# OpenResearchInstitute/ka9q-sdr

Hardware: AMD Instinct MI355X
Metric: input Msamples/s + channels @ real-time, 16384-pt overlap-save (higher is better)
Workload: dtype f32

## Files before the change

ka9q_sdr_amd/csrc/kq_bank.cpp:

```cpp
#include <cstdarg>

#include "kq_bank.hpp"

using namespace kq::bank;

namespace {
thread_local std::string g_err;

int ilog2(unsigned v) {
  int l = 0;
  while ((1u << l) < v) l++;
  return l;
}
}

void kq_internal_set_error(const char *fmt, ...) {
  char buf[512];
  va_list ap;
  va_start(ap, fmt);
  vsnprintf(buf, sizeof buf, fmt, ap);
  va_end(ap);
  g_err = buf;
}

// ... 235 lines not shown
      if (b->alloc(&h, C * (size_t)(g.Mdec > 1 ? g.Mdec - 1 : 1), true)) return -1;
  }
  if (b->alloc(&b->chd.foffset, C, true)) return -1;
  if (b->alloc(&b->chd.pdev, C, true)) return -1;
  if (b->alloc(&b->chd.gain, C, true)) return -1;
  if (b->alloc(&b->chd.hang, C, true)) return -1;
  if (b->alloc(&b->chd.dc, C, true)) return -1;
  if (b->alloc(&b->chd.n0, C, true)) return -1;
  if (b->alloc(&b->chd.pl_ptr, C, true)) return -1;
  if (b->alloc(&b->chd.pl_last, C, true)) return -1;
  if (b->alloc(&b->chd.plfreq, C, true)) return -1;
  if (g.pl_n > 0) {
    if (b->alloc(&b->chd.plresp, (size_t)g.pl_n / 2 + 1, true)) return -1;
    if (b->alloc(&b->chd.plring, C * 16384, true)) return -1;
  }
  if (b->alloc(&b->pl.audio, C * B * 2 * (size_t)g.olen, true)) return -1;
  if (b->alloc(&b->pl.status, C * B, true)) return -1;
  for (int k = 0; k < 2; k++) {
    b->pl2[k].audio = b->pl.audio;
    b->pl2[k].status = b->pl.status;
    if (b->alloc(&b->pl2[k].filt, C * B * g.olen, true)) return -1;
    if (b->alloc(&b->pl2[k].n0raw, C * B, true)) return -1;
    if (b->alloc(&b->pl2[k].if_power, B * (1 + kq::kEnergySplitMax), true)) return -1;
    if (g.pl_n > 0 && b->alloc(&b->pl2[k].plout, C * B * g.pl_l, true)) return -1;
  }
  b->pl = b->pl2[0];
  if (b->alloc(&b->energy_state, 2, true)) return -1;
  if (kq::full16k_paired_supported(g) && b->alloc(&b->win_paired, (size_t)(g.M - 1) + (size_t)B * g.L, true)) return -1;
  for (int *&l : b->list_dev)
    if (b->alloc(&l, C, true)) return -1;
  for (kq_bank::CtlQueue &q : b->ctl)
    for (int k = 0; k < kq_bank::CtlQueue::kDepth; k++)
      if (b->alloc_pinned(&q.buf[k], kq_bank::CtlQueue::kBytes) || b->new_event(&q.applied[k], hipEventDisableTiming)) return -1;
  {
    kq_bank::DesignQueue &d = b->dq;
    size_t const per_job = (size_t)g.Ndec * sizeof(float2);
    d.max_jobs = (unsigned)std::max<size_t>(1, std::min<size_t>(kq_bank::DesignQueue::kMax, ((size_t)64 << 20) / per_job));
    if (b->alloc(&d.scratch, (size_t)d.max_jobs * g.Ndec, true)) return -1;
    if (b->alloc(&d.ng_next, 2 * C, true)) return -1;
    for (int k = 0; k < kq_bank::DesignQueue::kDepth; k++)
      if (b->alloc_pinned(&d.pin[k], kq_bank::DesignQueue::kMax * (sizeof(kq::DesignJob) + sizeof(kq::DesignTarget))) ||
          b->new_event(&d.read[k], hipEventDisableTiming))
        return -1;
    for (hipEvent_t &e : d.ng_moved)
      if (b->new_event(&e, hipEventDisableTiming)) return -1;
    if (g.Ndec <= 16384 && kq::design_prepare(g.olen, g.Mdec)) return -1;
  }
  if (b->alloc(&b->list_active_dev, C, true)) return -1;
  if (b->alloc(&b->list_active_ds_dev, C, true)) return -1;
  if (b->alloc(&b->chd.fflags, C, true)) return -1;
  if (b->alloc(&b->list_unswept_dev, C, true)) return -1;
  if (b->alloc(&b->list_swept_dev, C, true)) return -1;
  if (b->fwd_mode == KQ_FWD_PRUNED && b->alloc(&b->chan_tw, C * kq::pruned_table_elems(g), true)) return -1;
  if (b->fwd_mode != KQ_FWD_PRUNED && kq::full16k_supported(g) && b->alloc(&b->chd.row_ph, C * 32, true)) return -1;
  KQ_TRY(hipStreamSynchronize(b->stream));
  if (g.pl_n > 0) {
    int const PL_M = g.pl_n - g.pl_l + 1;
    std::vector<kq::cfloat> r(g.pl_n / 2 + 1, kq::cfloat(0, 0));
    for (int j = 0; j <= g.pl_n / 2; j++) {
      float const f = (float)j * g.dsamprate / g.Ndec;
      if (f > 0 && f < 300) r[j] = 1;
    }
    if (kq::window_rfilter(g.pl_l, PL_M, r, 2.0)) return -1;
    KQ_TRY(hipMemcpy(b->chd.plresp, r.data(), r.size() * sizeof(float2), hipMemcpyHostToDevice));
  }
  {
    std::vector<float> nanv(C, NAN);
    KQ_TRY(hipMemcpy(b->chd.plfreq, nanv.data(), C * sizeof(float), hipMemcpyHostToDevice));
  }
  return 0;
}
}

kq_bank *kq_bank_create(const kq_bank_config *cfg) {
  if (create_check(cfg)) return nullptr;
  kq::DeviceScope dev_scope_(cfg->device);
  {
    int cur = -1;
    if (hipGetDevice(&cur) != hipSuccess || cur != cfg->device) {
      kq_internal_set_error("hipSetDevice(%d) failed", cfg->device);
      return nullptr;
    }
  }
  kq_bank *b = new kq_bank();
  b->cfg = *cfg;
  b->chans.reserve(cfg->max_channels);
  if (create_geometry(b) || create_alloc(b)) {
    kq_bank_destroy(b);
    return nullptr;
  }
  return b;
}

int kq_bank_destroy(kq_bank *b) {
  kq::DeviceScope dev_scope_(b ? b->cfg.device : -1);
  if (!b) return 0;
  b->close();
  delete b;
  return 0;
}

void *kq_bank_stream(kq_bank *b) { return b ? (void *)b->stream : nullptr; }

int kq_bank_join(kq_bank *b) {
  BankScope dev_scope_(b);
  if (!b) return -1;
  if (b->calls == 0) return 0;
// ... 59 lines not shown
```

ka9q_sdr_amd/csrc/kq_device.hpp:

```cpp
#pragma once
#include "kq_energy.hpp"
#include <hip/hip_runtime.h>
#include <stdint.h>

#include <functional>

#include "../../include/ka9q_hip.h"

struct filter_in;

namespace kq {

enum { FLAG_FLAT = 1, FLAG_ISB = 2, FLAG_STEREO = 4, FLAG_SQUARE = 8 };

struct PllState {
  double c_phase, c_freq;
  double f_phase, f_freq;
  float integrator, delta_f, snr, foffset, cphase;
  int lock_count, pll_lock, fft_samples, fft_ptr;
};

struct FftDim {
  int n;
  int log2n;
  int nf;
  unsigned char f[12];
  const unsigned short *rev;
  const float2 *twc;
  int tw_n;
};
FftDim fft_dim(int n, bool *ok);
bool fft_size_ok(int n);
const float2 *half_twiddles(int log2T);
enum { TABLE_HALF_TWIDDLES, TABLE_DIM_REV, TABLE_DIM_TW, TABLE_FULL16K };
const void *upload_once(int table, int size, size_t bytes, const std::function<void(void *)> &fill);

constexpr int kPllChunk = 64;
struct PllChunk {
  PllState *state;
  float2 *rings;
  float2 *side;
};

struct Geom {
  int N, L, M, D;
  FftDim dN, dNdec, dPl;
  int Ndec, olen, Mdec;
  int log2N, log2Ndec;
  int samprate;
  int tw_log2;
  int max_blocks;
  float dsamprate;
  int pl_n, pl_l;
};

constexpr int kOldLevels = 4;

struct ChanDev {
  int *mode;
  int *flags;
  int *fflags;
  float *low, *high;
  float2 *resp;
  float2 *aresp;
  float *fm_gain;
  float *headroom;
  float *recovery;
  int *hangmax;
  float *noise_gain;
  unsigned long long *n0lane;
  unsigned *n0meta;
  int *n0slot;
  double *lo_phase, *lo_freq, *lo_rate;
  float2 *row_ph;
  double *hist_phase, *hist_freq, *hist_rate;
  int *hist_len;
  int *hist2_len;
  double *hist2_osc;
  double *sh_phase, *sh_freq;
  float2 *fm_state;
  float *lastaudio;
  int *sq_count;
  float *ahist;
  float *foffset, *pdev;
  float *gain;
  int *hang;
  float *dc;
  float *n0;
  float2 *plresp;
  float *plring;
  int *pl_ptr, *pl_last;
  float *plfreq;
};

struct Planes {
  float2 *filt;
  float *audio;
  kq_chan_status *status;
  float *n0raw;
  float *if_power;
  float *plout;
};

struct DeviceScope {
  int prev = -1;
  bool switched = false;
  explicit DeviceScope(int device) {
    if (device < 0) return;
    if (hipGetDevice(&prev) == hipSuccess && prev != device) switched = hipSetDevice(device) == hipSuccess;
  }
  ~DeviceScope() {
    if (switched) (void)hipSetDevice(prev);
  }
  DeviceScope(const DeviceScope &) = delete;
  DeviceScope &operator=(const DeviceScope &) = delete;
};

void ensure_dynamic_lds(const void *kernel, size_t bytes);

void launch_copy_to_host(hipStream_t s, const float *audio, float *haudio, int row, const kq_chan_status *status, void *hstatus,
                         size_t rows);
void launch_copy_pcm_to_host(hipStream_t s, const float *audio, short *hpcm, unsigned *hmask, int row,
                             const kq_chan_status *status, void *hstatus, size_t rows, const int *mode_compact = nullptr,
                             int max_blocks = 1);
void launch_ingest(hipStream_t s, const void *src, int format, float2 *dst, size_t nsamples, float scale);
constexpr int kEnergySplitMax = 16;
int block_energy_split(int L);
// ... 68 lines not shown
```

ka9q_sdr_amd/csrc/kq_full16k.hip:

```cpp
#include "kq_device.hpp"
#include "kq_ldsfft.hpp"
#include <cmath>
#include <type_traits>

#include "kq_lane.hpp"
#include "kq_regfft.hpp"

#ifdef KQ_TIMELINE
__device__ unsigned long long kq_timeline[64][8][12];
#define KQ_STAMP(i)                                                                        \
  do {                                                                                     \
    __builtin_amdgcn_sched_barrier(0);                                                     \
    if (blockIdx.y == (gridDim.y > 40 ? 40 : gridDim.y / 2) && (blockIdx.x & 15) == 0 && (blockIdx.x >> 4) < 64 &&      \
        (threadIdx.x & 63) == 0)                                                           \
      kq_timeline[blockIdx.x >> 4][threadIdx.x >> 6][i] = clock64();                       \
    __builtin_amdgcn_sched_barrier(0);                                                     \
  } while (0)
extern "C" int kq_debug_timeline(unsigned long long *dst) {
  return hipMemcpyFromSymbol(dst, HIP_SYMBOL(kq_timeline), sizeof(kq_timeline)) == hipSuccess ? 0 : -1;
}
#else
#define KQ_STAMP(i)
#endif

namespace kq {

namespace {

constexpr int kN = 16384, kT = 512;
constexpr int kRow1 = 528;
constexpr int kCol2 = 32;
constexpr int kRow2 = 513;
constexpr int kXchElems = 16 * kRow1;

using rfft::pk_cmul;
using rfft::pk_cmul2;
using rfft::pk_cmul4;
using rfft::pk_cmul_s;
using rfft::v2f;

__device__ __forceinline__ v2f ld2(const float2 *p) {
  float2 const f = *p;
  return (v2f){f.x, f.y};
}

using rsrc_t = __amdgpu_buffer_rsrc_t;
__device__ __forceinline__ rsrc_t make_rsrc(const void *base, unsigned bytes) {
  return __builtin_amdgcn_make_buffer_rsrc(const_cast<void *>(base), 0, (int)bytes, 0x00020000);
}
__device__ __forceinline__ v2f buf_ld2(rsrc_t r, unsigned lane_off, unsigned row_off) {
  return __builtin_bit_cast(v2f, __builtin_amdgcn_raw_buffer_load_b64(r, (int)lane_off, (int)row_off, 0));
}
__device__ __forceinline__ void buf_ld4(v2f &a, v2f &b, rsrc_t r, unsigned lane_off, unsigned row_off) {
  typedef float v4f __attribute__((ext_vector_type(4)));
  v4f const q = __builtin_bit_cast(v4f, __builtin_amdgcn_raw_buffer_load_b128(r, (int)lane_off, (int)row_off, 0));
  a = (v2f){q.x, q.y};
  b = (v2f){q.z, q.w};
}

constexpr int kTabP1 = 0;
constexpr int kTabEpi = kTabP1 + 10 * kT;
constexpr int kTabTw2 = kTabEpi + 5 * 64, kTabSize = kTabTw2 + 512;
constexpr int kTw2Pitch = 34;

__device__ __forceinline__ void twiddle32(v2f (&v)[32], const v2f (&tlo)[3], const v2f (&thi)[7], v2f c) {
  v2f lo[4];
  lo[0] = c;
  pk_cmul2(lo[1], lo[2], c, tlo[0], c, tlo[1]);
  lo[3] = pk_cmul(c, tlo[2]);
  pk_cmul4(v[0], v[1], v[2], v[3], v[0], lo[0], v[1], lo[1], v[2], lo[2], v[3], lo[3]);
#pragma unroll
  for (int h = 1; h < 8; h++) {
    v2f w[4];
    pk_cmul4(w[0], w[1], w[2], w[3], thi[h - 1], lo[0], thi[h - 1], lo[1], thi[h - 1], lo[2], thi[h - 1], lo[3]);
    pk_cmul4(v[4 * h], v[4 * h + 1], v[4 * h + 2], v[4 * h + 3], v[4 * h], w[0], v[4 * h + 1], w[1], v[4 * h + 2], w[2],
             v[4 * h + 3], w[3]);
  }
}
__device__ __forceinline__ void twiddle32_fetch(v2f (&tlo)[3], v2f (&thi)[7], rsrc_t tab, int t) {
  v2f e[10];
#pragma unroll
  for (int j = 0; j < 5; j++) buf_ld4(e[2 * j], e[2 * j + 1], tab, (unsigned)t * 16u, (unsigned)(kTabP1 + 2 * kT * j) * 8u);
#pragma unroll
  for (int l = 0; l < 3; l++) tlo[l] = e[l];
#pragma unroll
  for (int h = 0; h < 7; h++) thi[h] = e[3 + h];
}

__device__ __forceinline__ v2f phasor2(double turns) {
  float2 const p = phasor_turns(turns);
  return (v2f){p.x, p.y};
}
__device__ __forceinline__ float2 row_phasor(double f0, int n1) { return phasor_turns(f0 * (double)(512 * n1)); }

constexpr double kSweepLimit64k = 1.1e-11;
constexpr double kSweepLimit16k = 4.8e-11;

__device__ __forceinline__ void sibling_exchange(unsigned long long *slots, int r4, unsigned value, unsigned tag, float *out,
                                                 int *err) {
  int const t = threadIdx.x;
  if (t == 0)
    __hip_atomic_store(slots + r4, ((unsigned long long)tag << 32) | value, __ATOMIC_RELAXED, __HIP_MEMORY_SCOPE_AGENT);
  if (t < 4) {
    unsigned long long w = 0;
    int it = 0;
    for (;;) {
      w = __hip_atomic_load(slots + t, __ATOMIC_RELAXED, __HIP_MEMORY_SCOPE_AGENT);
      if ((unsigned)(w >> 32) == tag || ++it > (1 << 18)) break;
      __builtin_amdgcn_s_sleep(8);
    }
    if ((unsigned)(w >> 32) != tag) {
      *err = 1;
      w = 0x7fc00000u;
    }
    out[t] = __uint_as_float((unsigned)w);
  }
  __syncthreads();
}

}

template <bool N0, bool DUMP, int PLAIN, bool PAIRED, int BIG, int EPI>
__global__ __launch_bounds__(kT, 4) void k_filter_full16k(Geom g, ChanDev ch, Planes pl, const float2 *__restrict__ window,
                                                       const float2 *__restrict__ tw, const float2 *__restrict__ tab,
                                                       float2 *__restrict__ spec_dump, int spec_ch,
                                                       const int *__restrict__ chan_list, Big64 big) {
  extern __shared__ __attribute__((aligned(16))) float2 xch[];
  constexpr bool kRowPlane = PLAIN == 1 && BIG == 0;
  __shared__ __attribute__((aligned(16))) float2 stab[kRowPlane ? 1 : (kT / 64) * (BIG ? 128 : 32)];
  __shared__ float sib_f[BIG ? 12 : 1];
  constexpr int kNfull = BIG ? 4 * kN : kN;
  int const r4 = BIG ? (int)(blockIdx.x & 3) : 0;
  __shared__ __attribute__((aligned(16))) float2 tw2[16 * kTw2Pitch];
  __shared__ float red_f[2][kT / 64];
  __shared__ float red_c[kT / 64];
  __shared__ int red_i[2][kT / 64];
  int const t = threadIdx.x;
  int const Ndec = g.Ndec;
  KQ_STAMP(0);
  __builtin_amdgcn_s_setprio(3);
  v2f v[32];
  rsrc_t const xr = make_rsrc(window + (size_t)blockIdx.y * g.L, kNfull * (unsigned)sizeof(float2));
  unsigned const toff = (unsigned)t * (unsigned)sizeof(float2);
  auto load_rows = [&](int first, int last) {
    if constexpr (PAIRED) {
#pragma unroll
      for (int n1 = first; n1 < last; n1 += 2)
        buf_ld4(v[rfft::bitrev5(n1)], v[rfft::bitrev5(n1 + 1)], xr, 2 * toff, (unsigned)(n1 / 2) * (unsigned)(1024 * sizeof(float2)));
    } else {
#pragma unroll
      for (int n1 = first; n1 < last; n1++) v[rfft::bitrev5(n1)] = buf_ld2(xr, toff, (unsigned)n1 * (unsigned)(512 * sizeof(float2)));
    }
  };
  auto load_window = [&]() { load_rows(0, 32); };
  rsrc_t const tabr = make_rsrc(tab, kTabSize * (unsigned)sizeof(float2));
  v2f tlo[3], thi[7];
  int const cidx = BIG ? (int)(blockIdx.x >> 2) : (int)blockIdx.x;
  int const c = chan_list ? chan_list[cidx] : cidx, b = blockIdx.y;
  v2f pt = (v2f){1.f, 0.f};
  if constexpr (BIG != 0) {
    double const ph0 = ch.lo_phase[c], f0 = ch.lo_freq[c], rs = ch.lo_rate[c];
    double const hp0 = ch.hist_phase[c], hf0 = ch.hist_freq[c], hr = ch.hist_rate[c];
    double const mbase = (double)b * g.L;
    int const n_old = (hp0 != ph0 || hf0 != f0 || hr != rs) ? ch.hist_len[c] - b * g.L : 0;
    bool const retuned = n_old > 0;
    if (PLAIN || (!retuned && fabs(rs) <= kSweepLimit64k)) {
      constexpr bool kSwept = !PLAIN || BIG == 2;
      v2f sa[2][4], sb[2][4];
      auto issue = [&](int i, int slot) {
#pragma unroll
        for (int j = 0; j < 4; j++) {
          if constexpr (PAIRED) {
            buf_ld4(sa[slot][j], sb[slot][j], xr, 2 * toff, (unsigned)(16 * j + i) * (unsigned)(1024 * sizeof(float2)));
          } else {
            sa[slot][j] = buf_ld2(xr, toff, (unsigned)(32 * j + 2 * i) * (unsigned)(512 * sizeof(float2)));
            sb[slot][j] = buf_ld2(xr, toff, (unsigned)(32 * j + 2 * i + 1) * (unsigned)(512 * sizeof(float2)));
          }
        }
      };
      issue(0, 0);
      issue(1, 1);
// ... 34 lines not shown
          v2f const w0[4] = {{tt[0].x, tt[0].y}, {tt[1].x, tt[1].y}, {tt[2].x, tt[2].y}, {tt[3].x, tt[3].y}};
          v2f const w1[4] = {{tt[0].z, tt[0].w}, {tt[1].z, tt[1].w}, {tt[2].z, tt[2].w}, {tt[3].z, tt[3].w}};
          pk_cmul2(zz[0], zz[1], sa[slot][0], w0[0], sb[slot][0], w1[0]);
#pragma unroll
          for (int j = 1; j < 4; j++) rfft::pk_cmadd2(zz[0], zz[1], sa[slot][j], w0[j], zz[0], sb[slot][j], w1[j], zz[1]);
        }
#pragma unroll
        for (int e = 0; e < 2; e++) {
          int const n1 = 2 * i + e;
          v2f x[4], w[4];
#pragma unroll
          for (int j = 0; j < 4; j++) {
            x[j] = e ? sb[slot][j] : sa[slot][j];
            w[j] = e ? (v2f){tt[j].z, tt[j].w} : (v2f){tt[j].x, tt[j].y};
          }
          v2f z;
          if constexpr (kSwept) {
            v2f y0, y1, y2, y3;
            pk_cmul4(y0, y1, y2, y3, x[0], w[0], x[1], w[1], x[2], w[2], x[3], w[3]);
            v2f const a = y1 + y3, bb = y2 + y3;
            v2f const S = (y0 + y2) + a;
            v2f const W = rfft::pk_fma(bb, (v2f){2.f, 2.f}, a);
            v2f const Uu = n1 ? rfft::pk_fma(S, (v2f){n1 / 32.f, n1 / 32.f}, W) : W;
            asm("v_pk_fma_f32 %0, %1, %2, %3 op_sel:[1,0,0] op_sel_hi:[0,1,1] neg_lo:[0,1,0]" : "=v"(z) : "v"(Uu), "v"(kb), "v"(S));
          } else {
            z = zz[e];
          }
          v[rfft::bitrev5(n1)] = z;
        }
        if (i + 2 < 16) issue(i + 2, slot);
      }
    } else {
      OlderOsc older;
      load_older(ch, c, b * g.L, n_old > 0, older);
#pragma unroll
      for (int n1 = 0; n1 < 32; n1++) {
        v2f acc = (v2f){0.f, 0.f};
        for (int j = 0; j < 4; j++) {
          int const i = 16384 * j + 512 * n1 + t;
          double const m = mbase + i;
          bool const old = i < n_old;
          double pp = old ? hp0 : ph0, ff = old ? hf0 : f0, rr = old ? hr : rs;
          pick_older(older, i, pp, ff, rr);
          double turns = pp + ff * m;
          if (rr != 0.0) turns += rr * (0.5 * m * (m - 1.0));
          turns -= (double)(r4 * (512 * n1 + t)) * (1.0 / 65536.0) + 0.25 * (double)(r4 * j);
          acc = rfft::pk_cmadd(buf_ld2(xr, toff, (unsigned)(32 * j + n1) * (unsigned)(512 * sizeof(float2))), phasor2(turns), acc);
        }
        v[rfft::bitrev5(n1)] = acc;
      }
    }
  }
  v2f srow[kRowPlane ? 32 : 1];
  if constexpr (PLAIN && BIG == 0) {
    double const ph0 = ch.lo_phase[c], f0 = ch.lo_freq[c];
    double const rs = PLAIN == 2 ? ch.lo_rate[c] : 0.0;
    if constexpr (kRowPlane) {
      typedef const float2 __attribute__((address_space(4))) *row_plane;
      row_plane const rp = (row_plane)(ch.row_ph + (size_t)__builtin_amdgcn_readfirstlane(c) * 32);
#pragma unroll
      for (int n1 = 1; n1 < 32; n1++) srow[n1] = (v2f){rp[n1].x, rp[n1].y};
    }
    load_rows(0, 12);
    __builtin_amdgcn_sched_barrier(0);
    if constexpr (PLAIN == 2) {
      float2 *const sw = stab + (t >> 6) * 32;
      if ((t & 63) < 32) {
        double const R = (double)(512 * (t & 63));
        double turns = f0 * R;
        turns += rs * (0.5 * R * (R - 1.0) + R * ((double)b * g.L + (double)(t & ~63)));
        sw[t & 63] = phasor_turns(turns);
      }
    }
    __builtin_amdgcn_sched_barrier(0);
    load_rows(12, 22);
    __builtin_amdgcn_sched_barrier(0);
    {
      double const A = (double)b * g.L + t;
      double turns = ph0 + f0 * A;
      if constexpr (PLAIN == 2) turns += rs * (0.5 * A * (A - 1.0));
      pt = phasor2(turns);
    }
    __builtin_amdgcn_sched_barrier(0);
    load_rows(22, 32);
  }
  twiddle32_fetch(tlo, thi, tabr, t);
  v2f const tw2_mine = buf_ld2(tabr, toff, (unsigned)kTabTw2 * 8u);
  KQ_STAMP(10);

  if constexpr (BIG == 0) {
    double const ph0 = ch.lo_phase[c], f0 = ch.lo_freq[c], r = ch.lo_rate[c];
    double const hp0 = ch.hist_phase[c], hf0 = ch.hist_freq[c], hr = ch.hist_rate[c];
    double const mbase = (double)b * g.L;
    int const n_old = (hp0 != ph0 || hf0 != f0 || hr != r) ? ch.hist_len[c] - b * g.L : 0;
    bool const retuned = n_old > 0;
    if (PLAIN || (r == 0.0 && !retuned)) {
      float2 *const sw = stab + (kRowPlane ? 0 : (t >> 6) * 32);
      if constexpr (!PLAIN) {
        load_window();
        if ((t & 63) < 32) sw[t & 63] = row_phasor(f0, t & 63);
        pt = phasor2(ph0 + f0 * (mbase + t));
      }
      KQ_STAMP(11);
      if constexpr (!kRowPlane) {
        __builtin_amdgcn_fence(__ATOMIC_RELEASE, "wavefront");
        __builtin_amdgcn_wave_barrier();
        __builtin_amdgcn_fence(__ATOMIC_ACQUIRE, "wavefront");
      }
      auto row = [&](int n1) -> v2f & { return v[rfft::bitrev5(n1)]; };
      auto mul = [&](auto firstc, auto countc, v2f(&y)[4]) {
        constexpr int n1 = decltype(firstc)::value, K = decltype(countc)::value;
        if constexpr (kRowPlane) {
          if constexpr (K == 4)
            rfft::pk_cmul_s4(y[0], y[1], y[2], y[3], row(n1), srow[n1], row(n1 + 1), srow[n1 + 1], row(n1 + 2), srow[n1 + 2],
                             row(n1 + 3), srow[n1 + 3]);
          else if constexpr (K == 2)
            rfft::pk_cmul_s2(y[0], y[1], row(n1), srow[n1], row(n1 + 1), srow[n1 + 1]);
          else
            y[0] = pk_cmul_s(row(n1), srow[n1]);
        } else {
          if constexpr (K == 4)
            pk_cmul4(y[0], y[1], y[2], y[3], row(n1), ld2(sw + n1), row(n1 + 1), ld2(sw + n1 + 1), row(n1 + 2), ld2(sw + n1 + 2),
                     row(n1 + 3), ld2(sw + n1 + 3));
          else if constexpr (K == 2)
            pk_cmul2(y[0], y[1], row(n1), ld2(sw + n1), row(n1 + 1), ld2(sw + n1 + 1));
          else
            y[0] = pk_cmul(row(n1), ld2(sw + n1));
        }
      };
      float const kbf = PLAIN == 2 ? (float)(2.0 * M_PI * 512.0 * r * (double)(t & 63)) : 0.f;
      v2f const kb = (v2f){kbf, kbf};
      v2f th = (v2f){0.f, 0.f};
      auto mix = [&](auto firstc, auto countc) {
        constexpr int n1 = decltype(firstc)::value, K = decltype(countc)::value;
        v2f y[4];
        mul(firstc, countc, y);
#pragma unroll
        for (int i = 0; i < K; i++) {
          if constexpr (PLAIN == 2) {
            th = th + kb;
            v2f z;
            asm("v_pk_fma_f32 %0, %1, %2, %3 op_sel:[1,0,0] op_sel_hi:[0,1,1] neg_lo:[0,1,0]" : "=v"(z) : "v"(y[i]), "v"(th), "v"(y[i]));
            row(n1 + i) = z;
          } else {
            row(n1 + i) = y[i];
          }
        }
      };
      using std::integral_constant;
      constexpr integral_constant<int, 1> k1{};
      constexpr integral_constant<int, 2> k2{};
      constexpr integral_constant<int, 4> k4{};
      mix(integral_constant<int, 1>{}, k1);
      mix(integral_constant<int, 2>{}, k2);
      mix(integral_constant<int, 4>{}, k4);
      mix(integral_constant<int, 8>{}, k4);
      mix(integral_constant<int, 12>{}, k4);
      mix(integral_constant<int, 16>{}, k4);
      mix(integral_constant<int, 20>{}, k2);
      mix(integral_constant<int, 22>{}, k2);
      mix(integral_constant<int, 24>{}, k4);
      mix(integral_constant<int, 28>{}, k4);
    } else if constexpr (!PLAIN) {
      OlderOsc older;
      load_older(ch, c, b * g.L, n_old > 0, older);
#pragma unroll
      for (int n1 = 0; n1 < 32; n1++) {
        int const i = 512 * n1 + t;
        double const m = mbase + i;
        bool const old = i < n_old;
        double pp = old ? hp0 : ph0, ff = old ? hf0 : f0, rr = old ? hr : r;
        pick_older(older, i, pp, ff, rr);
        double turns = pp + ff * m;
        if (rr != 0.0) turns += rr * (0.5 * m * (m - 1.0));
        v[rfft::bitrev5(n1)] = pk_cmul(buf_ld2(xr, toff, (unsigned)n1 * (unsigned)(512 * sizeof(float2))), phasor2(turns));
      }
    }
  }

  KQ_STAMP(1);
  __builtin_amdgcn_s_setprio(0);
  rfft::fft_dit_pk<32>(v);
  twiddle32(v, tlo, thi, pt);

  KQ_STAMP(2);
  v2f u[32];
  tw2[(t >> 5) * kTw2Pitch + (t & 31)] = make_float2(tw2_mine.x, tw2_mine.y);
#if defined(KQ_ABLATE) && (KQ_ABLATE & 1)
#pragma unroll
  for (int n2 = 0; n2 < 32; n2++) u[n2] = v[n2];
#else
  {
    int const rd = ((t >> 4) & 15) * kRow1 + (t & 15);
#pragma unroll
    for (int half = 0; half < 2; half++) {
#pragma unroll
      for (int k1 = 0; k1 < 16; k1++) xch[k1 * kRow1 + t] = make_float2(v[16 * half + k1].x, v[16 * half + k1].y);
#if !(defined(KQ_ABLATE) && (KQ_ABLATE & 4))
      __syncthreads();
#endif
      if ((t >> 8) == half) {
#pragma unroll
        for (int n2 = 0; n2 < 32; n2++) u[rfft::bitrev5(n2)] = ld2(xch + rd + 16 * n2);
      }
#if !(defined(KQ_ABLATE) && (KQ_ABLATE & 4))
      __syncthreads();
#endif
    }
  }
#endif

  KQ_STAMP(3);
  rfft::fft_dit_pk<32>(u);
  {
    const float4 *row = reinterpret_cast<const float4 *>(tw2 + (t & 15) * kTw2Pitch);
// ... 53 lines not shown
      o[kStep * (ka + 1024 * k3) + r4] = make_float2(ya[k3].x, ya[k3].y);
      o[kStep * (kb + 1024 * k3) + r4] = make_float2(yb[k3].x, yb[k3].y);
    }
  }

  KQ_STAMP(6);
  float2 *Xs = xch;
  float2 *G = Xs + Ndec;
  auto to_f2 = [](v2f a) { return make_float2(a.x, a.y); };
  if constexpr (BIG != 0) {
    float2 *const Xg = big.xs + ((size_t)c * g.max_blocks + b) * Ndec;
    auto put = [&](int q, v2f val) {
      int const k = 4 * q + r4;
      if (k <= Ndec / 2)
        Xg[k] = to_f2(val);
      else if (k > kNfull - Ndec / 2)
        Xg[k - kNfull + Ndec] = to_f2(val);
    };
    if (Ndec <= 4096) {
      put(ka, ya[0]);
      put(kb, yb[0]);
      put(ka + 15 * 1024, ya[15]);
      put(kb + 15 * 1024, yb[15]);
    } else {
#pragma unroll
      for (int k3 = 0; k3 < 16; k3++) {
        put(ka + 1024 * k3, ya[k3]);
        put(kb + 1024 * k3, yb[k3]);
      }
    }
  } else if (Ndec <= 1024) {
    if (ka <= Ndec / 2) Xs[ka] = to_f2(ya[0]);
    if (kb <= Ndec / 2) Xs[kb] = to_f2(yb[0]);
    if (ka + 15 * 1024 > kN - Ndec / 2) Xs[ka - 1024 + Ndec] = to_f2(ya[15]);
    if (kb + 15 * 1024 > kN - Ndec / 2) Xs[kb - 1024 + Ndec] = to_f2(yb[15]);
  } else {
#pragma unroll
    for (int k3 = 0; k3 < 16; k3++) {
      if (1024 * k3 > Ndec / 2 && 1024 * k3 + 1023 <= kN - Ndec / 2) continue;
#pragma unroll
      for (int half = 0; half < 2; half++) {
        int const n = (half ? kb : ka) + 1024 * k3;
        float2 const val = to_f2(half ? yb[k3] : ya[k3]);
        if (n <= Ndec / 2)
          Xs[n] = val;
        else if (n > kN - Ndec / 2)
          Xs[n - kN + Ndec] = val;
      }
    }
  }
  const float2 *H = ch.resp + (size_t)c * Ndec;
  bool const isb = (ch.fflags[c] & FLAG_ISB) != 0;
  v2f epi_h = {0.f, 0.f}, epi_h2 = {0.f, 0.f}, epi_w[5] = {};
  bool const epi64 = BIG == 0 && (EPI == 1 || (EPI == 0 && Ndec == 64));
  if (epi64 && t < 64) {
    int const q = (int)(__brev((unsigned)t) >> 26);
    epi_h = ld2(H + q);
    if (isb) epi_h2 = ld2(H + ((64 - q) & 63));
#pragma unroll
    for (int st = 0; st < 5; st++) epi_w[st] = buf_ld2(tabr, (unsigned)t * 8u, (unsigned)(kTabEpi + st * 64) * 8u);
  }
  int const epiR = (BIG == 0 && (EPI == 2 || (EPI == 0 && Ndec >= 128 && Ndec <= 512))) ? Ndec >> 6 : 0;
  v2f epi_post = {1.f, 0.f};
  if (epiR && t < 64 * epiR) {
    int const r = t >> 6, l = t & 63;
    int const q = (int)(__brev((unsigned)l) >> 26);
    int const k = epiR * q + r;
    epi_h = ld2(H + k);
    if (isb) epi_h2 = ld2(H + ((Ndec - k) & (Ndec - 1)));
#pragma unroll
    for (int st = 0; st < 5; st++) epi_w[st] = buf_ld2(tabr, (unsigned)l * 8u, (unsigned)(kTabEpi + st * 64) * 8u);
    float sn, cs;
    sincospif(2.f * (float)(r * l) / (float)Ndec, &sn, &cs);
    epi_post = (v2f){cs, sn};
  }

  bool n0_fast = false;
  int outside = 0;
  if constexpr (N0) {
    v2f pp[16];
    typedef const unsigned long long __attribute__((address_space(4))) *lane_masks;
    int const ns = __builtin_amdgcn_readfirstlane(ch.n0slot[c]);
    lane_masks const lm = (lane_masks)(
        ch.n0lane + ((size_t)(ns * (BIG ? 4 : 1) + r4) * (kT / 64) + __builtin_amdgcn_readfirstlane(t >> 6)) * 32);
#pragma unroll
    for (int k3 = 0; k3 < 16; k3++) {
      float p0, p1;
      asm("v_mul_f32 %0, %1, %1" : "=v"(p0) : "v"(ya[k3].x));
      asm("v_mul_f32 %0, %1, %1" : "=v"(p1) : "v"(yb[k3].x));
      asm("v_fma_f32 %0, %1, %1, %0" : "+v"(p0) : "v"(ya[k3].y));
      asm("v_fma_f32 %0, %1, %1, %0" : "+v"(p1) : "v"(yb[k3].y));
      asm("v_cndmask_b32_e64 %0, 0, %0, %1" : "+v"(p0) : "s"(lm[k3]));
      asm("v_cndmask_b32_e64 %0, 0, %0, %1" : "+v"(p1) : "s"(lm[16 + k3]));
      pp[k3] = (v2f){p0, p1};
    }
    outside = (int)ch.n0meta[ns * (BIG ? 4 : 1) + r4];
    v2f s2;
    {
      v2f const a0 = pp[0] + pp[1], a1 = pp[2] + pp[3], a2 = pp[4] + pp[5], a3 = pp[6] + pp[7];
      v2f const a4 = pp[8] + pp[9], a5 = pp[10] + pp[11], a6 = pp[12] + pp[13], a7 = pp[14] + pp[15];
      s2 = ((a0 + a1) + (a2 + a3)) + ((a4 + a5) + (a6 + a7));
    }
    float const tot = wave_sum_to63(s2.x + s2.y);
    if ((t & 63) == 63) red_f[0][t >> 6] = tot;
    __syncthreads();
    float total = 0;
#pragma unroll
    for (int k = 0; k < kT / 64; k++) total += red_f[0][k];
    int bins1 = outside;
    unsigned long long *const slots = BIG ? big.sync + ((size_t)c * g.max_blocks + b) * 12 : nullptr;
    if constexpr (BIG != 0) {
      sibling_exchange(slots, r4, __float_as_uint(total), big.epoch, sib_f, big.err);
      total = (sib_f[0] + sib_f[1]) + (sib_f[2] + sib_f[3]);
      const unsigned *const mt = ch.n0meta + ns * 4;
      bins1 = (int)(mt[0] + mt[1] + mt[2] + mt[3]);
    }
    float const thr = (total / bins1) * 2;
    n0_fast = total < INFINITY && thr < INFINITY && thr >= 1e-26f;
    if (n0_fast) {
      int const e = (__float_as_int(thr) >> 23) & 0xff;
      float const scale = __int_as_float((127 + 40 + 127 - e) << 23);
      float const cs = thr * scale;
      v2f const nsc = (v2f){-scale, -scale}, c2 = (v2f){cs, cs};
      v2f acc_e = (v2f){0.f, 0.f}, acc_o = acc_e, cnt_e = acc_e, cnt_o = acc_e;
#pragma unroll
      for (int k3 = 0; k3 < 16; k3++) {
        v2f keep;
// ... 43 lines not shown
          red_i[iter][t >> 6] = wave_bins;
        }
        __syncthreads();
        float tf = 0;
        int bins = 0;
#pragma unroll
        for (int k = 0; k < kT / 64; k++) {
          tf += red_f[iter][k];
          bins += red_i[iter][k];
        }
        if (BIG != 0 && iter == 0) {
          sibling_exchange(slots + 4, r4, __float_as_uint(tf), big.epoch, sib_f + 4, big.err);
          sibling_exchange(slots + 8, r4, (unsigned)bins, big.epoch, sib_f + 8, big.err);
          tf = (sib_f[4] + sib_f[5]) + (sib_f[6] + sib_f[7]);
          bins = (int)(__float_as_uint(sib_f[8]) + __float_as_uint(sib_f[9]) + __float_as_uint(sib_f[10]) + __float_as_uint(sib_f[11]));
        }
        avg = tf / bins;
        tf_last = tf;
        bins_last = bins;
      }
      if constexpr (BIG != 0) {
        if (t == 0) big.n0part[((size_t)c * g.max_blocks + b) * 4 + r4] = make_float2(tf_last, (float)bins_last);
      } else {
        if (t == 0) pl.n0raw[(size_t)c * g.max_blocks + b] = (float)(avg / (2.0 * kN * g.samprate));
      }
    }
  }

  KQ_STAMP(7);
  __syncthreads();
  KQ_STAMP(8);
  if (N0 && n0_fast && t == kT - 64) {
    float tf = 0, bins = 0;
#pragma unroll
    for (int k = 0; k < kT / 64; k++) {
      tf += red_f[1][k];
      bins += red_c[k];
    }
    bins -= (float)(kN - outside);
    if constexpr (BIG != 0) {
      big.n0part[((size_t)c * g.max_blocks + b) * 4 + r4] = make_float2(tf, bins);
    } else {
      float const avg = tf / bins;
      pl.n0raw[(size_t)c * g.max_blocks + b] = (float)(avg / (2.0 * kN * g.samprate));
    }
  }
  if (big.iir.sums != nullptr && blockIdx.x == 0 && blockIdx.y == 0 && t >= kT - 64)
    block_energy_iir_wave(big.iir.sums, big.iir.split, big.iir.update, big.iir.nblocks, big.iir.L, big.iir.state, big.iir.if_power,
                          t & 63);
  if constexpr (BIG != 0) return;
  if (epi64) {
    if (t >= 64) return;
    int const q = (int)(__brev((unsigned)t) >> 26);
    v2f z = pk_cmul(epi_h, ld2(Xs + q));
    if (isb && q != 0 && q != 32) {
      v2f const other = pk_cmul(epi_h2, ld2(Xs + 64 - q));
      v2f const oc = (v2f){other.x, -other.y};
      z = q < 32 ? z + oc : z - oc;
    }
    auto stage = [&](auto mm, v2f w, bool first) {
      constexpr int half = decltype(mm)::value;
      v2f const v = first ? z : pk_cmul(z, w);
      v2f const r = (v2f){lane_xor<half>(v.x, t), lane_xor<half>(v.y, t)};
      float const sg = __int_as_float(0x3f800000 | ((t & half) ? 0x80000000 : 0));
      z = rfft::pk_fma(v, (v2f){sg, sg}, r);
    };
    stage(std::integral_constant<int, 1>{}, z, true);
    stage(std::integral_constant<int, 2>{}, epi_w[0], false);
    stage(std::integral_constant<int, 4>{}, epi_w[1], false);
    stage(std::integral_constant<int, 8>{}, epi_w[2], false);
    stage(std::integral_constant<int, 16>{}, epi_w[3], false);
    stage(std::integral_constant<int, 32>{}, epi_w[4], false);
    float2 *o = pl.filt + ((size_t)c * g.max_blocks + b) * g.olen;
    if (t >= 64 - g.olen) o[t - (64 - g.olen)] = make_float2(z.x, z.y);
    KQ_STAMP(9);
    return;
  }
  if (epiR) {
    float2 *Z = G;
    if (t < 64 * epiR) {
      int const r = t >> 6, l = t & 63;
      int const q = (int)(__brev((unsigned)l) >> 26);
      int const k = epiR * q + r;
      v2f z = pk_cmul(epi_h, ld2(Xs + k));
      if (isb && k != 0 && 2 * k != Ndec) {
        v2f const other = pk_cmul(epi_h2, ld2(Xs + Ndec - k));
        v2f const oc = (v2f){other.x, -other.y};
        z = 2 * k < Ndec ? z + oc : z - oc;
      }
      auto stage = [&](auto mm, v2f w, bool first) {
        constexpr int half = decltype(mm)::value;
        v2f const v = first ? z : pk_cmul(z, w);
        v2f const rr = (v2f){lane_xor<half>(v.x, l), lane_xor<half>(v.y, l)};
        float const sg = __int_as_float(0x3f800000 | ((l & half) ? 0x80000000 : 0));
        z = rfft::pk_fma(v, (v2f){sg, sg}, rr);
      };
      stage(std::integral_constant<int, 1>{}, z, true);
      stage(std::integral_constant<int, 2>{}, epi_w[0], false);
      stage(std::integral_constant<int, 4>{}, epi_w[1], false);
      stage(std::integral_constant<int, 8>{}, epi_w[2], false);
      stage(std::integral_constant<int, 16>{}, epi_w[3], false);
      stage(std::integral_constant<int, 32>{}, epi_w[4], false);
      z = pk_cmul(z, epi_post);
      Z[64 * r + l] = make_float2(z.x, z.y);
    }
    __syncthreads();
    if (t >= 64) return;
    float2 *o = pl.filt + ((size_t)c * g.max_blocks + b) * g.olen;
    int const first = Ndec - g.olen;
    auto combine = [&](auto rc) {
      constexpr int R = decltype(rc)::value;
      constexpr int bits = R == 2 ? 1 : R == 4 ? 2 : 3;
      float2 v[R];
#pragma unroll
      for (int r = 0; r < R; r++) {
        float2 const zz = Z[64 * r + t];
        v[(int)(__brev((unsigned)r) >> (32 - bits))] = make_float2(zz.x, -zz.y);
      }
      rfft::fft_dit<R>(v);
#pragma unroll
      for (int j = 0; j < R; j++) {
        int const i = t + 64 * j - first;
        if (i >= 0 && i < g.olen) o[i] = make_float2(v[j].x, -v[j].y);
      }
    };
    if (epiR == 2)
      combine(std::integral_constant<int, 2>{});
    else if (epiR == 4)
      combine(std::integral_constant<int, 4>{});
    else
      combine(std::integral_constant<int, 8>{});
    KQ_STAMP(9);
    return;
  }
  if constexpr (EPI != 0) return;
  for (int p = t; p <= Ndec / 2; p += kT) {
    float2 gp = cmul(H[p], Xs[p]);
    if (p > 0 && p < Ndec / 2) {
      int const k = Ndec - p;
      float2 gn = cmul(H[k], Xs[k]);
      if (isb) {
        float2 const pos = gp, neg = gn;
        gp = cadd(pos, cconj(neg));
        gn = csub(neg, cconj(pos));
      }
      G[bitrev((unsigned)k, g.log2Ndec)] = gn;
    }
    G[bitrev((unsigned)p, g.log2Ndec)] = gp;
  }
  lds_fft<+1>(G, g.log2Ndec, tw, g.tw_log2);

  float2 *o = pl.filt + ((size_t)c * g.max_blocks + b) * g.olen;
  for (int i = t; i < g.olen; i += kT) o[i] = G[Ndec - g.olen + i];
  KQ_STAMP(9);
}

__global__ void k_epilogue64k(Geom g, ChanDev ch, Planes pl, const float2 *__restrict__ tw, Big64 big,
                              const int *__restrict__ chan_list, int compute_n0) {
  extern __shared__ __attribute__((aligned(16))) float2 G[];
  int const t = threadIdx.x, Ndec = g.Ndec;
  int const c = chan_list ? chan_list[blockIdx.x] : (int)blockIdx.x, b = blockIdx.y;
  size_t const cb = (size_t)c * g.max_blocks + b;
  if (compute_n0 && t == 0) {
    const float2 *p = big.n0part + cb * 4;
    float const tf = (p[0].x + p[1].x) + (p[2].x + p[3].x), bins = (p[0].y + p[1].y) + (p[2].y + p[3].y);
    float const avg = tf / bins;
    pl.n0raw[cb] = (float)(avg / (2.0 * 65536.0 * g.samprate));
  }
  const float2 *Xs = big.xs + cb * Ndec;
  const float2 *H = ch.resp + (size_t)c * Ndec;
  bool const isb = (ch.fflags[c] & FLAG_ISB) != 0;
  for (int p = t; p <= Ndec / 2; p += blockDim.x) {
    float2 gp = cmul(H[p], Xs[p]);
    if (p > 0 && p < Ndec / 2) {
      int const k = Ndec - p;
      float2 gn = cmul(H[k], Xs[k]);
      if (isb) {
        float2 const pos = gp, neg = gn;
        gp = cadd(pos, cconj(neg));
        gn = csub(neg, cconj(pos));
      }
      G[bitrev((unsigned)k, g.log2Ndec)] = gn;
    }
    G[bitrev((unsigned)p, g.log2Ndec)] = gp;
  }
  lds_fft<+1>(G, g.log2Ndec, tw, g.tw_log2);
  float2 *o = pl.filt + cb * g.olen;
  for (int i = t; i < g.olen; i += blockDim.x) o[i] = G[Ndec - g.olen + i];
}

__global__ void __launch_bounds__(256) k_full16k_rows(ChanDev ch, int nchan) {
  int const i = (int)(blockIdx.x * blockDim.x + threadIdx.x);
  if (i >= 32 * nchan) return;
  ch.row_ph[i] = row_phasor(ch.lo_freq[i >> 5], i & 31);
}
void launch_full16k_rows(hipStream_t s, const ChanDev &ch, int nchan) {
  if (nchan > 0 && ch.row_ph) hipLaunchKernelGGL(k_full16k_rows, dim3((32 * nchan + 255) / 256), dim3(256), 0, s, ch, nchan);
}

bool full16k_supported(const Geom &g) {
  return g.N == kN && 2 * g.Ndec <= kXchElems && g.Ndec >= 4;
}

static const float2 *twiddle_tables() {
  return (const float2 *)upload_once(TABLE_FULL16K, kN, kTabSize * sizeof(float2), [](void *bytes) {
    float2 *h = (float2 *)bytes;
    auto w = [](long long e) {
      double const ang = -2.0 * M_PI * (double)(e % kN) / kN;
      return make_float2((float)cos(ang), (float)sin(ang));
    };
    for (int t = 0; t < kT; t++)
      for (int e = 0; e < 10; e++)
        h[kTabP1 + 2 * (kT * (e >> 1) + t) + (e & 1)] = e < 3 ? w((long long)(e + 1) * t) : w(4LL * (e - 2) * t);
    for (int n3 = 0; n3 < 16; n3++)
      for (int k2 = 0; k2 < 32; k2++) h[kTabTw2 + 32 * n3 + k2] = w(32LL * n3 * k2);
    for (int st = 1; st <= 5; st++)
      for (int t = 0; t < 64; t++) {
        int const half = 1 << st;
        double const ang = M_PI * (double)(t & (half - 1)) / half;
        h[kTabEpi + (st - 1) * 64 + t] = (t & half) ? make_float2((float)cos(ang), (float)sin(ang)) : make_float2(1.f, 0.f);
      }
  });
}

bool full16k_paired_supported(const Geom &g) {
  return (full16k_supported(g) || full64k_supported(g)) && g.L % 1024 == 0 && (g.M - 1) % 1024 == 0;
}

bool full64k_supported(const Geom &g) { return g.N == 4 * kN && g.Ndec >= 4 && g.Ndec <= 16384; }
double full64k_sweep_limit() { return kSweepLimit64k; }
double full16k_sweep_limit() { return kSweepLimit16k; }

void launch_filter_full16k(hipStream_t s, const Geom &g, const ChanDev &ch, const Planes &pl, const float2 *window,
                           const float2 *tw, int nchan, int nblocks, int compute_n0, float2 *spec_dump, int spec_ch,
                           const int *chan_list, int plain, const float2 *window_paired, const Big64 &big) {
  size_t const lds_bytes = (size_t)kXchElems * sizeof(float2);
  const float2 *tab = twiddle_tables();
  if (!tab) {
    launch_filter_full(s, g, ch, pl, window, tw, nchan, nblocks, compute_n0, spec_dump, spec_ch, chan_list);
    if (big.iir.sums)
      launch_block_energy_iir(s, big.iir.sums, big.iir.L, big.iir.nblocks, big.iir.update, big.iir.state, big.iir.if_power);
    return;
  }
  bool const n0 = compute_n0 && ch.n0lane && ch.n0meta;
  bool const dump = spec_dump != nullptr;
  if (plain == 1 && !ch.row_ph) plain = 0;
  bool const paired = plain && window_paired != nullptr;
  auto go = [&](auto kernel) {
    ensure_dynamic_lds((const void *)kernel, lds_bytes);
    hipLaunchKernelGGL(kernel, dim3(nchan, nblocks), dim3(kT), lds_bytes, s, g, ch, pl, paired ? window_paired : window, tw, tab,
                       spec_dump, spec_ch, chan_list, big);
  };
  int const epi = dump ? 0 : g.Ndec == 64 ? 1 : (g.Ndec >= 128 && g.Ndec <= 512) ? 2 : 0;
  auto pick3 = [&](auto n0c, auto dumpc, auto epic) {
    constexpr bool kN0 = decltype(n0c)::value, kDump = decltype(dumpc)::value;
    constexpr int kEpi = decltype(epic)::value;
    if (plain == 2)
      paired ? go(k_filter_full16k<kN0, kDump, 2, true, 0, kEpi>) : go(k_filter_full16k<kN0, kDump, 2, false, 0, kEpi>);
    else if (paired)
      go(k_filter_full16k<kN0, kDump, 1, true, 0, kEpi>);
    else
      plain ? go(k_filter_full16k<kN0, kDump, 1, false, 0, kEpi>) : go(k_filter_full16k<kN0, kDump, 0, false, 0, kEpi>);
  };
  auto pick = [&](auto n0c, auto dumpc) {
    if constexpr (decltype(dumpc)::value) {
      pick3(n0c, dumpc, std::integral_constant<int, 0>{});
    } else {
      if (epi == 1)
        pick3(n0c, dumpc, std::integral_constant<int, 1>{});
      else if (epi == 2)
        pick3(n0c, dumpc, std::integral_constant<int, 2>{});
      else
        pick3(n0c, dumpc, std::integral_constant<int, 0>{});
    }
  };
  using T = std::true_type;
  using F = std::false_type;
  if (n0)
    dump ? pick(T{}, T{}) : pick(T{}, F{});
  else
    dump ? pick(F{}, T{}) : pick(F{}, F{});
}

void launch_filter_full64k(hipStream_t s, const Geom &g, const ChanDev &ch, const Planes &pl, const float2 *window,
                           const float2 *tw, int nchan, int nblocks, int compute_n0, float2 *spec_dump, int spec_ch,
                           const int *chan_list, bool plain, bool swept, const float2 *window_paired, const Big64 &big) {
  size_t const lds_bytes = (size_t)kXchElems * sizeof(float2);
  const float2 *tab = twiddle_tables();
  if (!tab) {
    if (big.iir.sums)
      launch_block_energy_iir(s, big.iir.sums, big.iir.L, big.iir.nblocks, big.iir.update, big.iir.state, big.iir.if_power);
    return;
  }
  bool const n0 = compute_n0 && ch.n0lane && ch.n0meta;
  bool const dump = spec_dump != nullptr;
  bool const paired = plain && window_paired != nullptr;
  auto go = [&](auto kernel) {
    ensure_dynamic_lds((const void *)kernel, lds_bytes);
    hipLaunchKernelGGL(kernel, dim3(4 * nchan, nblocks), dim3(kT), lds_bytes, s, g, ch, pl, paired ? window_paired : window, tw,
// ... 25 lines not shown
```

Before: 386,100.

## Factor LO phasor into precomputed lane/wave tables and defer block phase to epilogue

Each thread's double-precision LO phasor evaluation is split into factors. Per-channel lane and wave phasors are precomputed into a new col_ph table by the rows kernel, and per-thread they are combined with a single complex multiply. The per-block phase factor is deferred, when allowed, to the small epilogue where it multiplies only the output bins instead of every input sample. This removes per-sample double-precision sincos work from the hot front-end, at the cost of an extra table and some float rounding from chaining products.

```diff
diff --git a/ka9q_sdr_amd/csrc/kq_bank.cpp b/ka9q_sdr_amd/csrc/kq_bank.cpp
--- a/ka9q_sdr_amd/csrc/kq_bank.cpp
+++ b/ka9q_sdr_amd/csrc/kq_bank.cpp
@@ -311,7 +311,9 @@
   if (b->alloc(&b->list_unswept_dev, C, true)) return -1;
   if (b->alloc(&b->list_swept_dev, C, true)) return -1;
   if (b->fwd_mode == KQ_FWD_PRUNED && b->alloc(&b->chan_tw, C * kq::pruned_table_elems(g), true)) return -1;
-  if (b->fwd_mode != KQ_FWD_PRUNED && kq::full16k_supported(g) && b->alloc(&b->chd.row_ph, C * 32, true)) return -1;
+  if (b->fwd_mode != KQ_FWD_PRUNED && kq::full16k_supported(g) &&
+      (b->alloc(&b->chd.row_ph, C * 32, true) || b->alloc(&b->chd.col_ph, C * kq::kFull16kColPitch, true)))
+    return -1;
   KQ_TRY(hipStreamSynchronize(b->stream));
   if (g.pl_n > 0) {
     int const PL_M = g.pl_n - g.pl_l + 1;
diff --git a/ka9q_sdr_amd/csrc/kq_device.hpp b/ka9q_sdr_amd/csrc/kq_device.hpp
--- a/ka9q_sdr_amd/csrc/kq_device.hpp
+++ b/ka9q_sdr_amd/csrc/kq_device.hpp
@@ -54,6 +54,7 @@
   int pl_n, pl_l;
 };
 
+constexpr int kFull16kColPitch = 72;
 constexpr int kOldLevels = 4;
 
 struct ChanDev {
@@ -73,6 +74,7 @@
   int *n0slot;
   double *lo_phase, *lo_freq, *lo_rate;
   float2 *row_ph;
+  float2 *col_ph;
   double *hist_phase, *hist_freq, *hist_rate;
   int *hist_len;
   int *hist2_len;
diff --git a/ka9q_sdr_amd/csrc/kq_full16k.hip b/ka9q_sdr_amd/csrc/kq_full16k.hip
--- a/ka9q_sdr_amd/csrc/kq_full16k.hip
+++ b/ka9q_sdr_amd/csrc/kq_full16k.hip
@@ -28,6 +28,7 @@
 namespace {
 
 constexpr int kN = 16384, kT = 512;
+constexpr int kColPitch = kFull16kColPitch;
 constexpr int kRow1 = 528;
 constexpr int kCol2 = 32;
 constexpr int kRow2 = 513;
@@ -92,6 +93,12 @@
   return (v2f){p.x, p.y};
 }
 __device__ __forceinline__ float2 row_phasor(double f0, int n1) { return phasor_turns(f0 * (double)(512 * n1)); }
+__device__ __forceinline__ float2 lane_phasor(double f0, int l) { return phasor_turns(f0 * (double)l); }
+__device__ __forceinline__ float2 wave_phasor(double f0, int w) { return phasor_turns(f0 * (double)(64 * w)); }
+__device__ __forceinline__ float2 block_phasor(double ph0, double f0, int b, int L) {
+  return phasor_turns(ph0 + f0 * ((double)b * L));
+}
+__device__ __forceinline__ v2f f2v(float2 p) { return (v2f){p.x, p.y}; }
 
 constexpr double kSweepLimit64k = 1.1e-11;
 constexpr double kSweepLimit16k = 4.8e-11;
@@ -127,6 +134,8 @@
                                                        const int *__restrict__ chan_list, Big64 big) {
   extern __shared__ __attribute__((aligned(16))) float2 xch[];
   constexpr bool kRowPlane = PLAIN == 1 && BIG == 0;
+  constexpr bool kDefer = BIG == 0 && PLAIN != 2 && EPI != 0 && !DUMP;
+  bool deferred = false;
   __shared__ __attribute__((aligned(16))) float2 stab[kRowPlane ? 1 : (kT / 64) * (BIG ? 128 : 32)];
   __shared__ float sib_f[BIG ? 12 : 1];
   constexpr int kNfull = BIG ? 4 * kN : kN;
@@ -267,18 +276,21 @@
     }
   }
   v2f srow[kRowPlane ? 32 : 1];
+  v2f swave = (v2f){1.f, 0.f}, vlane = (v2f){1.f, 0.f}, bfront = (v2f){1.f, 0.f};
   if constexpr (PLAIN && BIG == 0) {
-    double const ph0 = ch.lo_phase[c], f0 = ch.lo_freq[c];
-    double const rs = PLAIN == 2 ? ch.lo_rate[c] : 0.0;
     if constexpr (kRowPlane) {
       typedef const float2 __attribute__((address_space(4))) *row_plane;
-      row_plane const rp = (row_plane)(ch.row_ph + (size_t)__builtin_amdgcn_readfirstlane(c) * 32);
+      int const cu = __builtin_amdgcn_readfirstlane(c);
+      row_plane const rp = (row_plane)(ch.row_ph + (size_t)cu * 32);
 #pragma unroll
       for (int n1 = 1; n1 < 32; n1++) srow[n1] = (v2f){rp[n1].x, rp[n1].y};
+      row_plane const cp = (row_plane)(ch.col_ph + (size_t)cu * kColPitch + 64 + __builtin_amdgcn_readfirstlane(t >> 6));
+      swave = (v2f){cp[0].x, cp[0].y};
     }
     load_rows(0, 12);
     __builtin_amdgcn_sched_barrier(0);
     if constexpr (PLAIN == 2) {
+      double const f0 = ch.lo_freq[c], rs = ch.lo_rate[c];
       float2 *const sw = stab + (t >> 6) * 32;
       if ((t & 63) < 32) {
         double const R = (double)(512 * (t & 63));
@@ -290,14 +302,20 @@
     __builtin_amdgcn_sched_barrier(0);
     load_rows(12, 22);
     __builtin_amdgcn_sched_barrier(0);
-    {
+    if constexpr (PLAIN == 2) {
+      double const ph0 = ch.lo_phase[c], f0 = ch.lo_freq[c], rs = ch.lo_rate[c];
       double const A = (double)b * g.L + t;
       double turns = ph0 + f0 * A;
-      if constexpr (PLAIN == 2) turns += rs * (0.5 * A * (A - 1.0));
+      turns += rs * (0.5 * A * (A - 1.0));
       pt = phasor2(turns);
+    } else if constexpr (!kDefer) {
+      bfront = f2v(block_phasor(ch.lo_phase[c], ch.lo_freq[c], b, g.L));
     }
     __builtin_amdgcn_sched_barrier(0);
     load_rows(22, 32);
+    if constexpr (kRowPlane)
+      vlane = buf_ld2(make_rsrc(ch.col_ph + (size_t)__builtin_amdgcn_readfirstlane(c) * kColPitch, 64 * (unsigned)sizeof(float2)),
+                      toff & (63u * (unsigned)sizeof(float2)), 0);
   }
   twiddle32_fetch(tlo, thi, tabr, t);
   v2f const tw2_mine = buf_ld2(tabr, toff, (unsigned)kTabTw2 * 8u);
@@ -314,8 +332,10 @@
       if constexpr (!PLAIN) {
         load_window();
         if ((t & 63) < 32) sw[t & 63] = row_phasor(f0, t & 63);
-        pt = phasor2(ph0 + f0 * (mbase + t));
-      }
+        pt = pk_cmul(f2v(lane_phasor(f0, t & 63)), f2v(wave_phasor(f0, t >> 6)));
+        if constexpr (!kDefer) pt = pk_cmul(pt, f2v(block_phasor(ph0, f0, b, g.L)));
+      }
+      deferred = kDefer;
       KQ_STAMP(11);
       if constexpr (!kRowPlane) {
         __builtin_amdgcn_fence(__ATOMIC_RELEASE, "wavefront");
@@ -376,6 +396,10 @@
       mix(integral_constant<int, 22>{}, k2);
       mix(integral_constant<int, 24>{}, k4);
       mix(integral_constant<int, 28>{}, k4);
+      if constexpr (kRowPlane) {
+        pt = pk_cmul_s(vlane, swave);
+        if constexpr (!kDefer) pt = pk_cmul(pt, bfront);
+      }
     } else if constexpr (!PLAIN) {
       OlderOsc older;
       load_older(ch, c, b * g.L, n_old > 0, older);
@@ -535,6 +559,7 @@
   const float2 *H = ch.resp + (size_t)c * Ndec;
   bool const isb = (ch.fflags[c] & FLAG_ISB) != 0;
   v2f epi_h = {0.f, 0.f}, epi_h2 = {0.f, 0.f}, epi_w[5] = {};
+  v2f epi_b = {1.f, 0.f};
   bool const epi64 = BIG == 0 && (EPI == 1 || (EPI == 0 && Ndec == 64));
   if (epi64 && t < 64) {
     int const q = (int)(__brev((unsigned)t) >> 26);
@@ -542,6 +567,7 @@
     if (isb) epi_h2 = ld2(H + ((64 - q) & 63));
 #pragma unroll
     for (int st = 0; st < 5; st++) epi_w[st] = buf_ld2(tabr, (unsigned)t * 8u, (unsigned)(kTabEpi + st * 64) * 8u);
+    if (kDefer && deferred) epi_b = f2v(block_phasor(ch.lo_phase[c], ch.lo_freq[c], b, g.L));
   }
   int const epiR = (BIG == 0 && (EPI == 2 || (EPI == 0 && Ndec >= 128 && Ndec <= 512))) ? Ndec >> 6 : 0;
   v2f epi_post = {1.f, 0.f};
@@ -556,6 +582,7 @@
     float sn, cs;
     sincospif(2.f * (float)(r * l) / (float)Ndec, &sn, &cs);
     epi_post = (v2f){cs, sn};
+    if (kDefer && deferred) epi_b = f2v(block_phasor(ch.lo_phase[c], ch.lo_freq[c], b, g.L));
   }
 
   bool n0_fast = false;
@@ -705,9 +732,10 @@
   if (epi64) {
     if (t >= 64) return;
     int const q = (int)(__brev((unsigned)t) >> 26);
-    v2f z = pk_cmul(epi_h, ld2(Xs + q));
+    auto bin = [&](int k) { return (kDefer && deferred) ? pk_cmul(epi_b, ld2(Xs + k)) : ld2(Xs + k); };
+    v2f z = pk_cmul(epi_h, bin(q));
     if (isb && q != 0 && q != 32) {
-      v2f const other = pk_cmul(epi_h2, ld2(Xs + 64 - q));
+      v2f const other = pk_cmul(epi_h2, bin(64 - q));
       v2f const oc = (v2f){other.x, -other.y};
       z = q < 32 ? z + oc : z - oc;
     }
@@ -735,9 +763,10 @@
       int const r = t >> 6, l = t & 63;
       int const q = (int)(__brev((unsigned)l) >> 26);
       int const k = epiR * q + r;
-      v2f z = pk_cmul(epi_h, ld2(Xs + k));
+      auto bin = [&](int kk) { return (kDefer && deferred) ? pk_cmul(epi_b, ld2(Xs + kk)) : ld2(Xs + kk); };
+      v2f z = pk_cmul(epi_h, bin(k));
       if (isb && k != 0 && 2 * k != Ndec) {
-        v2f const other = pk_cmul(epi_h2, ld2(Xs + Ndec - k));
+        v2f const other = pk_cmul(epi_h2, bin(Ndec - k));
         v2f const oc = (v2f){other.x, -other.y};
         z = 2 * k < Ndec ? z + oc : z - oc;
       }
@@ -842,13 +871,22 @@
   for (int i = t; i < g.olen; i += blockDim.x) o[i] = G[Ndec - g.olen + i];
 }
 
+constexpr int kRowEvals = 32 + kFull16kColPitch;
 __global__ void __launch_bounds__(256) k_full16k_rows(ChanDev ch, int nchan) {
   int const i = (int)(blockIdx.x * blockDim.x + threadIdx.x);
-  if (i >= 32 * nchan) return;
-  ch.row_ph[i] = row_phasor(ch.lo_freq[i >> 5], i & 31);
+  if (i >= kRowEvals * nchan) return;
+  int const c = i / kRowEvals, e = i - kRowEvals * c;
+  double const f0 = ch.lo_freq[c];
+  if (e < 32)
+    ch.row_ph[32 * c + e] = row_phasor(f0, e);
+  else if (e < 96)
+    ch.col_ph[kFull16kColPitch * c + (e - 32)] = lane_phasor(f0, e - 32);
+  else
+    ch.col_ph[kFull16kColPitch * c + (e - 32)] = wave_phasor(f0, e - 96);
 }
 void launch_full16k_rows(hipStream_t s, const ChanDev &ch, int nchan) {
-  if (nchan > 0 && ch.row_ph) hipLaunchKernelGGL(k_full16k_rows, dim3((32 * nchan + 255) / 256), dim3(256), 0, s, ch, nchan);
+  if (nchan > 0 && ch.row_ph && ch.col_ph)
+    hipLaunchKernelGGL(k_full16k_rows, dim3((kRowEvals * nchan + 255) / 256), dim3(256), 0, s, ch, nchan);
 }
 
 bool full16k_supported(const Geom &g) {
@@ -897,7 +935,7 @@
   }
   bool const n0 = compute_n0 && ch.n0lane && ch.n0meta;
   bool const dump = spec_dump != nullptr;
-  if (plain == 1 && !ch.row_ph) plain = 0;
+  if (plain == 1 && !(ch.row_ph && ch.col_ph)) plain = 0;
   bool const paired = plain && window_paired != nullptr;
   auto go = [&](auto kernel) {
     ensure_dynamic_lds((const void *)kernel, lds_bytes);
```

Measured after the change: 389,300, median of 6. About the same (+0.8%).
